# EvolEcolGroup/tidypopgen

Measured on AMD Instinct MI355X. Metric: SNP-genotypes/s (N x M) for IBS+KING+GRM+Fst+PCA; max |delta| vs CPU ref (cpu_baseline.parity), higher is better.
Workload: dtype fp4-e2m1 operands (exact integers, f32 accumulate) for the cross-products, the PCA Gram and the grouped counts, int8 (int32 accumulate) for the loadings, f64 for statistics

## Files before the change

include/tpg.h:

```cpp
#ifndef TPG_H
#define TPG_H

#include <stddef.h>
#include <stdint.h>

#ifdef __cplusplus
extern "C" {
#endif

#define TPG_OK 0
#define TPG_EINVAL 1
#define TPG_EHIP 2
#define TPG_EUNSUPPORTED 3
#define TPG_ENUMERIC 4

typedef struct tpg_ctx tpg_ctx;
typedef struct tpg_fbm tpg_fbm;
typedef struct tpg_view tpg_view;
typedef struct tpg_pairwise tpg_pairwise;
typedef struct tpg_comm tpg_comm;
typedef struct tpg_multi tpg_multi;

const char* tpg_last_error(void);
const char* tpg_version(void);
// ... 473 lines not shown
  int32_t* loci_counts;
  double* hwe_p;
  int32_t* grouped_counts;
  double* grouped_hwe_p;
  int32_t* indiv_counts;
} tpg_stream_qc_job;
int tpg_stream_qc(tpg_ctx* ctx, tpg_stream* s, const tpg_stream_qc_job* job, tpg_stream_report* report);

int tpg_pca_center_scale(tpg_ctx* ctx, const tpg_view* v, double* center, double* scale);
int tpg_pca_gram(tpg_ctx* ctx, const tpg_view* v, const double* center, const double* scale, double* K);
int tpg_pca_gram_add(tpg_ctx* ctx, const tpg_view* v, const double* center, const double* scale, double* K);
int tpg_pca_partial_svd(tpg_ctx* ctx, const tpg_view* v, int k, double* d, double* u, double* vload,
                        double* center, double* scale, double* square_frobenius);
int tpg_pca_random_svd(tpg_ctx* ctx, const tpg_view* v, int k, double tol, double* d, double* u, double* vload,
                       double* center, double* scale, double* square_frobenius);
int tpg_sym_eig_topk(tpg_ctx* ctx, const double* K, int64_t n, int k, double* lambda, double* U);
int tpg_pca_loadings(tpg_ctx* ctx, const tpg_view* v, const double* center, const double* scale,
                     const double* U, const double* d, int k, double* vload);
int tpg_fbm256_prod_and_rowSumsSq(tpg_ctx* ctx, const tpg_view* v, const double* center,
                                  const double* scale, const double* V, int K, double* XV, double* rss);
int tpg_square_frobenius(tpg_ctx* ctx, const tpg_view* v, const double* center, const double* scale,
                         double* out);
int tpg_fbm256_valid_prod(tpg_ctx* ctx, const tpg_view* v, const double* Tab, int K, double* out);

#define TPG_PCA_OP_TOL_FLOOR 1e-8
int tpg_pca_zt_prod(tpg_ctx* ctx, const tpg_view* v, const double* center, const double* scale, const double* Q, int b,
                    double* W);
int tpg_pca_z_prod(tpg_ctx* ctx, const tpg_view* v, const double* center, const double* scale, const double* W, int b,
                   double* Y);
int tpg_pca_random_svd_op(tpg_ctx* ctx, const tpg_view* v, int k, double tol, double* d, double* u, double* vload,
                          double* center, double* scale, double* square_frobenius, int* n_apply);
size_t tpg_pca_op_scratch_bytes(int64_t n, int64_t m, int k);
int tpg_pca_gram_route_fits(tpg_ctx* ctx, int64_t n, int k, int* fits);

#define TPG_PCADAPT_MAX_K 64
#define TPG_SELECT_TILE 1024
int64_t tpg_select_tile(void);
int tpg_col_median_mad(tpg_ctx* ctx, const double* X, int64_t rows, int ncols, int64_t ld, double* med, double* mad,
                       int64_t* n_finite);
int tpg_pcadapt_zscores(tpg_ctx* ctx, const tpg_view* v, const double* U, int K, double* z, int64_t* n_valid);
int tpg_robust_dist_ogk(tpg_ctx* ctx, const double* Z, int64_t m, int K, double* dist, double* center, double* cov,
                        double* basis, int64_t* n_valid);
int tpg_pchisq_log10_upper(tpg_ctx* ctx, const double* x, int64_t count, int df, double* out);
int tpg_qchisq_median(int df, double* out);
int tpg_pcadapt(tpg_ctx* ctx, const tpg_view* v, const double* U, int K, double* z, double* dist, double* stat, double* log10p,
                double* gc_lambda, int64_t* n_valid);

int tpg_view_select_loci(tpg_ctx* ctx, const tpg_view* v, const int64_t* idx0, int64_t count, tpg_view** out);
int tpg_qnorm_upper(double p, double* x);
int tpg_rollmean_weights(int radius, double* w);
int tpg_rollmean_segments(tpg_ctx* ctx, const double* x, int64_t m, const int64_t* seg_start, int64_t nseg, int radius,
                          double* out);
int tpg_medcouple(tpg_ctx* ctx, const double* x, int64_t count, double* mc);
#define TPG_TUKEY_REPORT_DOUBLES 7
int tpg_tukey_mc_up(tpg_ctx* ctx, const double* x, int64_t count, double alpha, double* report);
int tpg_pca_auto_svd(tpg_ctx* ctx, const tpg_view* v, const int32_t* chrom, const int64_t* hi, int k, double thr_r2, int roll_size,
                     double alpha_tukey, int64_t min_mac, int max_iter, void** out);
int64_t tpg_autosvd_count(const void* r);
int tpg_autosvd_iters(const void* r);
int tpg_autosvd_converged(const void* r);
int tpg_autosvd_fetch(const void* r, double* d, double* u, double* vload, double* center, double* scale, int64_t* idx0,
                      double* square_frobenius);
int tpg_autosvd_history(const void* r, int iter, int64_t* n_kept, int64_t* n_outliers, double* report);
int tpg_autosvd_outliers(const void* r, int iter, int64_t* pos0, int64_t* idx0);
int tpg_autosvd_intervals(const void* r, int iter, int64_t min_size, int64_t* first0, int64_t* last0, int64_t* count);
void tpg_autosvd_free(void* r);
// ... 61 lines not shown
```

tidypopgen_amd/_lib.py:

```python
from __future__ import annotations

import ctypes as C
import os

_HERE = os.path.dirname(os.path.abspath(__file__))
LIB_PATH = os.environ.get("TPG_LIB_PATH") or os.path.join(_HERE, "libtpg_hip.so")


class TpgError(RuntimeError):
    def __init__(self, code: int, msg: str):
        super().__init__(f"[tpg error {code}] {msg}")
        self.code = code


def build(force: bool = False) -> str:
    import subprocess

    csrc = os.path.join(_HERE, "csrc")
    cmd = ["make", "-C", csrc, "-j8", "-s"]
    if force:
        cmd.append("-B")
    subprocess.check_call(cmd)
    return LIB_PATH

# ... 246 lines not shown
    "tpg_multi_create": (ci, [ci, vp, vp]),
    "tpg_multi_destroy": (None, [vp]),
    "tpg_multi_ndev": (ci, [vp]),
    "tpg_multi_ctx": (vp, [vp, ci]),
    "tpg_multi_comm": (vp, [vp, ci]),
    "tpg_multi_pairwise": (ci, [vp, vp, i64, i64, vp, i64, vp, i64, ci, vp, vp, vp, vp]),
    "tpg_multi_grouped_alt_freq": (ci, [vp, vp, i64, i64, vp, i64, vp, i64, vp, vp, ci, vp, ci, vp]),
    "tpg_multi_pop_fst": (ci, [vp, vp, i64, i64, vp, i64, vp, i64, vp, vp, ci, vp, ci, vp, ci, ci, ci, vp, vp, vp]),
    "tpg_multi_pca_partial_svd": (ci, [vp, vp, i64, i64, vp, i64, vp, i64, vp, ci, vp, vp, vp, vp, vp, vp]),
    "tpg_stream_open_host": (ci, [vp, vp, i64, i64, sz, vp]),
    "tpg_stream_open_bk": (ci, [vp, cstr, i64, i64, sz, vp]),
    "tpg_stream_open_bed": (ci, [vp, cstr, i64, i64, sz, vp]),
    "tpg_stream_open_bed_host": (ci, [vp, vp, i64, i64, sz, vp]),
    "tpg_stream_open_synth": (ci, [vp, u64, i64, i64, ci, u32, ci, sz, vp]),
    "tpg_stream_close": (None, [vp]),
    "tpg_stream_run": (ci, [vp, vp, P(StreamJob), P(StreamReport)]),
    "tpg_multi_stream_run": (ci, [vp, vp, P(StreamJob), P(StreamReport)]),
    "tpg_stream_qc": (ci, [vp, vp, P(StreamQcJob), P(StreamReport)]),
    "tpg_pca_center_scale": (ci, [vp, vp, vp, vp]),
    "tpg_pca_gram": (ci, [vp, vp, vp, vp, vp]),
    "tpg_pca_gram_add": (ci, [vp, vp, vp, vp, vp]),
    "tpg_pca_partial_svd": (ci, [vp, vp, ci, vp, vp, vp, vp, vp, vp]),
    "tpg_pca_random_svd": (ci, [vp, vp, ci, f64, vp, vp, vp, vp, vp, vp]),
    "tpg_sym_eig_topk": (ci, [vp, vp, i64, ci, vp, vp]),
    "tpg_pca_loadings": (ci, [vp, vp, vp, vp, vp, vp, ci, vp]),
    "tpg_fbm256_prod_and_rowSumsSq": (ci, [vp, vp, vp, vp, vp, ci, vp, vp]),
    "tpg_square_frobenius": (ci, [vp, vp, vp, vp, vp]),
    "tpg_fbm256_valid_prod": (ci, [vp, vp, vp, ci, vp]),
    "tpg_pca_zt_prod": (ci, [vp, vp, vp, vp, vp, ci, vp]),
    "tpg_pca_z_prod": (ci, [vp, vp, vp, vp, vp, ci, vp]),
    "tpg_pca_random_svd_op": (ci, [vp, vp, ci, f64, vp, vp, vp, vp, vp, vp, vp]),
    "tpg_pca_op_scratch_bytes": (sz, [i64, i64, ci]),
    "tpg_pca_gram_route_fits": (ci, [vp, i64, ci, vp]),
    "tpg_select_tile": (i64, []),
    "tpg_col_median_mad": (ci, [vp, vp, i64, ci, i64, vp, vp, vp]),
    "tpg_pcadapt_zscores": (ci, [vp, vp, vp, ci, vp, vp]),
    "tpg_robust_dist_ogk": (ci, [vp, vp, i64, ci, vp, vp, vp, vp, vp]),
    "tpg_pchisq_log10_upper": (ci, [vp, vp, i64, ci, vp]),
    "tpg_qchisq_median": (ci, [ci, vp]),
    "tpg_pcadapt": (ci, [vp, vp, vp, ci, vp, vp, vp, vp, vp, vp]),
    "tpg_view_select_loci": (ci, [vp, vp, vp, i64, vp]),
    "tpg_qnorm_upper": (ci, [f64, vp]),
    "tpg_rollmean_weights": (ci, [ci, vp]),
    "tpg_rollmean_segments": (ci, [vp, vp, i64, vp, i64, ci, vp]),
    "tpg_medcouple": (ci, [vp, vp, i64, vp]),
    "tpg_tukey_mc_up": (ci, [vp, vp, i64, f64, vp]),
    "tpg_pca_auto_svd": (ci, [vp, vp, vp, vp, ci, f64, ci, f64, i64, ci, vp]),
    "tpg_autosvd_count": (i64, [vp]),
    "tpg_autosvd_iters": (ci, [vp]),
    "tpg_autosvd_converged": (ci, [vp]),
    "tpg_autosvd_fetch": (ci, [vp, vp, vp, vp, vp, vp, vp, vp]),
    "tpg_autosvd_history": (ci, [vp, ci, vp, vp, vp]),
    "tpg_autosvd_outliers": (ci, [vp, ci, vp, vp]),
    "tpg_autosvd_intervals": (ci, [vp, ci, i64, vp, vp, vp]),
    "tpg_autosvd_free": (None, [vp]),
    "tpg_kmeans_chunk_doubles": (i64, []),
    "tpg_kmeans_start": (ci, [u64, i64, ci, vp]),
    "tpg_kmeans_step": (ci, [vp, vp, i64, ci, ci, vp, vp, vp, vp, vp]),
    "tpg_kmeans_batch": (ci, [vp, vp, i64, ci, ci, vp, vp, ci, vp, vp, vp, vp, vp, vp, vp]),
    "tpg_cluster_wss": (ci, [vp, vp, i64, ci, ci, vp, vp, vp, vp]),
    "tpg_hclust_ward": (ci, [vp, vp, i64, ci, ci, vp, vp, vp]),
    "tpg_hclust_ward_trace": (ci, [vp, vp, i64, ci, ci, vp, vp, vp, vp]),
    "tpg_hclust_cut": (ci, [i64, vp, vp, ci, vp, vp]),
    "tpg_hclust_r_merge": (ci, [i64, vp, vp, vp]),
    "tpg_lda": (ci, [vp, i64, ci, vp, ci, ci, vp, vp, vp, vp, vp, vp, vp, vp, vp, vp, vp]),
    "tpg_dapc_var_contr": (ci, [vp, vp, i64, i64, ci, vp, ci, vp, vp]),
# ... 27 lines not shown
```

tidypopgen_amd/csrc/gramcls.hip:

```cpp
#include <math.h>
#include <string.h>

#include <algorithm>
#include <vector>

#include <hipcub/hipcub.hpp>

#include "common.h"
#include "devfrag.h"
#include "host/host_bits2.h"

constexpr int GA = 2, GB = 2, GP = GA * GB;
#define GCLS_SLAB (GP * 16 * 64)
#define GCLS_MAX_RUN 65536

__global__ void tpg_gcls_keys_kernel(const double* __restrict__ w, int64_t m, unsigned long long* __restrict__ key,
                                     uint32_t* __restrict__ idx) {
  for (int64_t j = blockIdx.x * (int64_t)blockDim.x + threadIdx.x; j < m; j += (int64_t)gridDim.x * blockDim.x) {
    const unsigned long long b = (unsigned long long)__double_as_longlong(w[j]);
    key[j] = (b + 16ull) & ~31ull;
    idx[j] = (uint32_t)j;
  }
}

__global__ void tpg_gcls_run_blocks_kernel(const uint32_t* __restrict__ counts, const int* __restrict__ nruns, int64_t m,
                                           uint32_t* __restrict__ cnt_out, uint32_t* __restrict__ nblk) {
  const int nr = nruns[0];
  for (int64_t r = blockIdx.x * (int64_t)blockDim.x + threadIdx.x; r < m; r += (int64_t)gridDim.x * blockDim.x) {
    const uint32_t c = r < nr ? counts[r] : 0u;
    cnt_out[r] = c;
    nblk[r] = (c + 63u) / 64u;
  }
}

__device__ __forceinline__ int tpg_gcls_find_run(const uint32_t* __restrict__ start, int nr, uint32_t x) {
  int lo = 0, hi = nr - 1;
  while (lo < hi) {
    const int mid = (lo + hi + 1) >> 1;
    if (start[mid] <= x) lo = mid; else hi = mid - 1;
  }
  return lo;
}

// ... 155 lines not shown
    __builtin_amdgcn_wave_barrier();
    __builtin_amdgcn_fence(__ATOMIC_ACQUIRE, "workgroup");
#pragma unroll
    for (int s = 0; s < 4; s++) {
      uint4 o = rd_dst[s * (2 * GSH_HS / 4)];
      if constexpr (CEN) {
        const uint32_t A[2] = {o.x, o.y}, B[2] = {o.z, o.w};
        uint32_t out[4];
#pragma unroll
        for (int t = 0; t < 2; t++) {
          const uint32_t nb = ~B[t], lo = nb & v55[t], hi = (nb >> 1) & lo, bc = lo | (hi << 1);
          out[2 * t] = (A[t] & 0x33333333u) | ((bc & 0x33333333u) << 2);
          out[2 * t + 1] = ((A[t] >> 2) & 0x33333333u) | (bc & 0xCCCCCCCCu);
        }
        o = make_uint4(out[0], out[1], out[2], out[3]);
      }
      T2g[((4 * q + s) * rs2 + bp) * 64 + lane] = o;
    }
    __builtin_amdgcn_fence(__ATOMIC_RELEASE, "workgroup");
    __builtin_amdgcn_wave_barrier();
    }
#pragma unroll
    for (int hb = 0; hb < 2; hb++) {
#pragma unroll
      for (int qi = 0; qi < QW; qi++) { w[qi][hb][0] = wn[qi][hb][0]; w[qi][hb][1] = wn[qi][hb][1]; }
      j0[hb] = j1[hb]; j1[hb] = j2[hb];
    }
  }
}

#define GCLS_SC_TWO ((int)0x80808080)

#define GCLS_D 2
__global__ __launch_bounds__(256, 2) void tpg_gcls_gram_kernel(const uint4* __restrict__ T2g, int64_t nblocks, int64_t rs2, int nrtv,
                                                               const unsigned long long* __restrict__ wblk,
                                                               const int2* __restrict__ order, int64_t nun, int S,
                                                               double* __restrict__ slabs) {
  constexpr int WPE = 2;
  const int lane = threadIdx.x & 63;
  const int wv = __builtin_amdgcn_readfirstlane(threadIdx.x >> 6);
  const int hgrid = gridDim.x / WPE, half = (int)blockIdx.x / hgrid, bx = (int)blockIdx.x % hgrid;
  const int xcd = bx & 7, cidx = bx >> 3, cpx = hgrid >> 3;
  const int SH = S / WPE;
  const int64_t npairs = (nblocks + 1) >> 1;
  for (int64_t round = 0;; round++) {
    const int64_t un = ((round * 8 + xcd) * cpx + cidx) * 4 + wv;
    if (un >= nun * SH) break;
    const int ks = half * SH + (int)(un / nun);
    const int64_t u = un % nun;
    const int2 ijv = order[u];
    const int2 ij = make_int2(__builtin_amdgcn_readfirstlane(ijv.x), __builtin_amdgcn_readfirstlane(ijv.y));
    const int64_t p0 = tpg_uniform64((npairs * ks) / S), p1 = tpg_uniform64((npairs * (ks + 1)) / S);
    const int64_t bend = 2 * p1 < nblocks ? 2 * p1 : nblocks;
    const uint4* pt[GA + GB];
#pragma unroll
    for (int t = 0; t < GA; t++) pt[t] = T2g + ((int64_t)min(GA * ij.x + t, nrtv - 1) * rs2) * 64;
#pragma unroll
    for (int t = 0; t < GB; t++) pt[GA + t] = T2g + ((int64_t)min(GB * ij.y + t, nrtv - 1) * rs2) * 64;

    double o[GP][16];
#pragma unroll
    for (int p = 0; p < GP; p++)
#pragma unroll
      for (int i = 0; i < 16; i++) o[p][i] = 0.0;
    v16f acc[GP];
#pragma unroll
    for (int p = 0; p < GP; p++)
#pragma unroll
      for (int i = 0; i < 16; i++) acc[p][i] = 0.f;

    if (p0 < p1) {
      const int64_t pl = p1 - 1, bl = bend - 1;
      v4u R[GCLS_D][GA + GB];
      auto LD = [&](const uint4* p) {
        uint32_t off = (uint32_t)lane * 16u;
        asm("" : "+v"(off));
        return *(const v4u*)((const char*)p + off);
      };
      tpg_static_for<GCLS_D - 1>([&](auto dd) {
        constexpr int d = decltype(dd)::value;
        const int64_t pc = p0 + d < p1 ? p0 + d : pl;
#pragma unroll
        for (int t = 0; t < GA + GB; t++) R[d][t] = LD(pt[t] + pc * 64);
      });
      bool first = true;
// ... 12 lines not shown
              const int64_t b = 2 * pr + hb;
              if (b < bend) {
                const unsigned long long wf = wf_next;
                wf_next = wblk[b < bl ? b + 1 : bl];
                v4u X[GA + GB];
#pragma unroll
                for (int t = 0; t < GA + GB; t++) {
                  const uint32_t w0 = R[C][t][2 * hb], w1 = R[C][t][2 * hb + 1];
                  X[t] = v4u{w0 & 0x33333333u, (w0 >> 2) & 0x33333333u, w1 & 0x33333333u, (w1 >> 2) & 0x33333333u};
                }
                if (first) {
                  const v16f z = {0, 0, 0, 0, 0, 0, 0, 0, 0, 0, 0, 0, 0, 0, 0, 0};
#pragma unroll
                  for (int p = 0; p < GP; p++) acc[p] = tpg_mfma_f4(X[p / GB], X[GA + p % GB], z, GCLS_SC_TWO, GCLS_SC_TWO);
                } else {
#pragma unroll
                  for (int p = 0; p < GP; p++) acc[p] = tpg_mfma_f4(X[p / GB], X[GA + p % GB], acc[p], GCLS_SC_TWO, GCLS_SC_TWO);
                }
                first = false;
                if ((wf & 1ull) || b == bl) {
                  const double w = __longlong_as_double((long long)(wf & ~1ull));
#pragma unroll
                  for (int p = 0; p < GP; p++)
#pragma unroll
                    for (int i = 0; i < 16; i++) o[p][i] = __builtin_fma((double)acc[p][i], w, o[p][i]);
                  first = true;
                }
              }
            }
          }
        });
      }
    }
    double* slab = slabs + ((int64_t)ks * nun + u) * GCLS_SLAB + lane;
#pragma unroll
    for (int p = 0; p < GP; p++)
#pragma unroll
      for (int i = 0; i < 16; i++) slab[(p * 16 + i) * 64] = o[p][i];
  }
}

typedef float v2f __attribute__((ext_vector_type(2)));
#define GCLS2_T_CLASS 0.045
#define GCLS2_T_BLOCK 0.067
#define GCLS2_LDS_BYTES (4 * 2 * 16 * 64 * 8)
#ifndef GCLS2_D
#define GCLS2_D 2
#endif
#define GCLS_SC_HALF ((int)0x7E7E7E7E)
template <bool CEN>
__global__ __launch_bounds__(256, 2) void tpg_gcls_gram2_kernel(const uint4* __restrict__ T2g, int64_t nblocks, int64_t rs2, int nrtv,
                                                                const ulonglong2* __restrict__ wblk,
                                                                const int2* __restrict__ order, int64_t nun, int S,
                                                                double* __restrict__ slabs) {
  extern __shared__ double olds_raw[];
  constexpr int WPE = 2;
  const int lane = threadIdx.x & 63;
  const int wv = __builtin_amdgcn_readfirstlane(threadIdx.x >> 6);
  double* olds = olds_raw + (size_t)wv * (2 * 16 * 64) + lane;
  const int hgrid = gridDim.x / WPE, half = (int)blockIdx.x / hgrid, bx = (int)blockIdx.x % hgrid;
  const int xcd = bx & 7, cidx = bx >> 3, cpx = hgrid >> 3;
  const int SH = S / WPE;
  const int64_t npairs = (nblocks + 1) >> 1;
  for (int64_t round = 0;; round++) {
    const int64_t un = ((round * 8 + xcd) * cpx + cidx) * 4 + wv;
    if (un >= nun * SH) break;
    const int ks = half * SH + (int)(un / nun);
    const int64_t u = un % nun;
    const int2 ijv = order[u];
    const int2 ij = make_int2(__builtin_amdgcn_readfirstlane(ijv.x), __builtin_amdgcn_readfirstlane(ijv.y));
    const int p0 = __builtin_amdgcn_readfirstlane((int)((npairs * ks) / S)), p1 = __builtin_amdgcn_readfirstlane((int)((npairs * (ks + 1)) / S));
    const int bend = 2 * p1;
    const char* pt[GA + GB];
#pragma unroll
    for (int t = 0; t < GA; t++) pt[t] = (const char*)(T2g + ((int64_t)min(GA * ij.x + t, nrtv - 1) * rs2 + p0) * 64);
#pragma unroll
    for (int t = 0; t < GB; t++) pt[GA + t] = (const char*)(T2g + ((int64_t)min(GB * ij.y + t, nrtv - 1) * rs2 + p0) * 64);

    double o[2][16];
    v2f dev[GP][8];
    v16f acc[GP];
#pragma unroll
    for (int p = 0; p < GP; p++) {
#pragma unroll
      for (int i = 0; i < 16; i++) acc[p][i] = 0.f;
#pragma unroll
      for (int i = 0; i < 8; i++) dev[p][i] = v2f{0.f, 0.f};
    }
#pragma unroll
    for (int p = 0; p < 2; p++)
#pragma unroll
      for (int i = 0; i < 16; i++) { o[p][i] = 0.0; olds[(p * 16 + i) * 64] = 0.0; }

    if (p0 < p1) {
      const int pl = p1 - 1, bl = bend - 1;
      v4u R[GCLS2_D][GA + GB];
      auto LDP = [&](v4u* slot, int pc) {
        uint32_t off = (uint32_t)lane * 16u + (uint32_t)(pc - p0) * 1024u;
        asm("" : "+v"(off));
#pragma unroll
        for (int t = 0; t < GA + GB; t++) slot[t] = *(const v4u*)(pt[t] + off);
      };
      tpg_static_for<GCLS2_D - 1>([&](auto dd) {
        constexpr int d = decltype(dd)::value;
// ... 84 lines not shown
                    for (int e = 0; e < 4; e++) dev[pr_][(e0 >> 1) + e] = dev[pl_][(e0 >> 1) + e] = v2f{0.f, 0.f};
                    __builtin_amdgcn_sched_barrier(0);
                  });
                } else {
                  pdelta = __uint_as_float((uint32_t)wf.y);
                  st = 2;
                }
                }
              }
            }
          }
        });
      }
      {
        const double w = __longlong_as_double((long long)(wlast & ~3ull));
        tpg_static_for<4>([&](auto hh) {
          constexpr int h = decltype(hh)::value, pr_ = h >> 1, pl_ = 2 + (h >> 1), e0 = (h & 1) * 8;
          double t[8];
#pragma unroll
          for (int e = 0; e < 8; e++) t[e] = olds[((pl_ - 2) * 16 + e0 + e) * 64];
#pragma unroll
          for (int e = 0; e < 8; e++) {
            const int i = e0 + e;
            o[pr_][i] = __builtin_fma((double)acc[pr_][i], w, o[pr_][i]) + (double)dev[pr_][i >> 1][i & 1];
          }
#pragma unroll
          for (int e = 0; e < 8; e++) {
            const int i = e0 + e;
            olds[((pl_ - 2) * 16 + i) * 64] = __builtin_fma((double)acc[pl_][i], w, t[e]) + (double)dev[pl_][i >> 1][i & 1];
          }
        });
      }
    }
    double* slab = slabs + ((int64_t)ks * nun + u) * GCLS_SLAB + lane;
#pragma unroll
    for (int p = 0; p < GP; p++)
#pragma unroll
      for (int i = 0; i < 16; i++) slab[(p * 16 + i) * 64] = p < 2 ? o[p][i] : olds[((p - 2) * 16 + i) * 64];
  }
}

__global__ __launch_bounds__(256) void tpg_gcls_assemble_kernel(const double* __restrict__ slabs, const int2* __restrict__ order,
                                                                int64_t nun, int S, int n, double* __restrict__ K) {
  __shared__ double tile[GP][32][33];
  const int lane = threadIdx.x & 63, wv = threadIdx.x >> 6;
  static_assert(GP == 4, "one wave per tile of the unit");
  for (int64_t u = blockIdx.x; u < nun; u += gridDim.x) {
    const int2 ij = order[u];
    const int p = wv;
    const int ti = GA * ij.x + p / GB, tk = GB * ij.y + p % GB;
    if (tk < ti) continue;
    double v[16];
#pragma unroll
    for (int reg = 0; reg < 16; reg++) v[reg] = 0.0;
    for (int s = 0; s < S; s++) {
      const double* sl = slabs + ((int64_t)s * nun + u) * GCLS_SLAB + (p * 16) * 64 + lane;
#pragma unroll
      for (int reg = 0; reg < 16; reg++) v[reg] += sl[reg * 64];
    }
#pragma unroll
    for (int reg = 0; reg < 16; reg++) tile[p][tpg_cd_row(reg, lane)][lane & 31] = v[reg];
    __builtin_amdgcn_fence(__ATOMIC_RELEASE, "workgroup");
    __builtin_amdgcn_wave_barrier();
    __builtin_amdgcn_fence(__ATOMIC_ACQUIRE, "workgroup");
    const int a = lane & 31, h = lane >> 5;
#pragma unroll 4
    for (int it = 0; it < 16; it++) {
      const int c = 2 * it + h;
      const int i1 = 32 * ti + a, k1 = 32 * tk + c;
      if (i1 < n && k1 < n) K[i1 + (int64_t)k1 * n] = tile[p][a][c];
      const int i2 = 32 * ti + c, k2 = 32 * tk + a;
      if (i2 < n && k2 < n) K[k2 + (int64_t)i2 * n] = tile[p][c][a];
    }
    __builtin_amdgcn_wave_barrier();
  }
}

static bool gcls_fold64(int64_t nruns, int64_t nblocks) {
  if (tpg_env_set("TPG_GRAM_FOLD64")) return tpg_env_int("TPG_GRAM_FOLD64", 0) != 0;
  return (double)nruns < 0.15 * (double)nblocks;
}

static double gcls_cost_classes(int64_t nunits, int64_t nruns, int64_t nblocks, int nwaves, int* bestS) {
  double best = -1;
  const bool f64 = gcls_fold64(nruns, nblocks);
  const double t_class = f64 ? 0.136 : GCLS2_T_CLASS, t_block = f64 ? 0.079 : GCLS2_T_BLOCK;
  for (int S = 2; S <= 32; S += 2) {
    if (nblocks / S < 4 && S > 2) break;
    const int64_t rounds = ceil_div(nunits * S, (int64_t)nwaves);
    const double per = ((double)nruns / S + 1.0) * GP * t_class + (double)ceil_div(nblocks, (int64_t)S) * GP * t_block + 6.0;
    const double cost = (double)rounds * per + (double)S * (double)nunits * 8.5e-3;
    if (best < 0 || cost < best * 0.995) { best = cost; *bestS = S; }
  }
  return best;
}

static int gram_classes_core(tpg_ctx* ctx, int64_t n, int64_t Q, int64_t m, const GclsSrc& src, const double* d_w, double* d_what,
                             double* d_K, bool force, bool* done, bool centred_ok) {
  *done = false;
  if (m >= (1ll << 31) - 64 || (tpg_env_set("TPG_GRAM_DIGITS") && !force)) return TPG_OK;
  DevArena B;
  unsigned long long *d_key = nullptr, *d_key2 = nullptr, *d_ukeys = nullptr;
  uint32_t *d_idx = nullptr, *d_idx2 = nullptr, *d_counts = nullptr, *d_cnt = nullptr, *d_nblk = nullptr, *d_estart = nullptr,
           *d_bstart = nullptr;
  int* d_nruns = nullptr;
  long long* d_totals = nullptr;
  void* d_tmp = nullptr;
  TPG_TRY(B.get(&d_key, (size_t)m)); TPG_TRY(B.get(&d_key2, (size_t)m)); TPG_TRY(B.get(&d_ukeys, (size_t)m));
  TPG_TRY(B.get(&d_idx, (size_t)m)); TPG_TRY(B.get(&d_idx2, (size_t)m)); TPG_TRY(B.get(&d_counts, (size_t)m));
  TPG_TRY(B.get(&d_cnt, (size_t)m)); TPG_TRY(B.get(&d_nblk, (size_t)m)); TPG_TRY(B.get(&d_estart, (size_t)m));
  TPG_TRY(B.get(&d_bstart, (size_t)m)); TPG_TRY(B.get(&d_nruns, 1)); TPG_TRY(B.get(&d_totals, 2));
  size_t t_sort = 0, t_rle = 0, t_scan = 0;
  TPG_HIP(hipcub::DeviceRadixSort::SortPairs(nullptr, t_sort, d_key, d_key2, d_idx, d_idx2, (int)m, 0, 64, ctx->stream));
  TPG_HIP(hipcub::DeviceRunLengthEncode::Encode(nullptr, t_rle, d_key2, d_ukeys, d_counts, d_nruns, (int)m, ctx->stream));
  TPG_HIP(hipcub::DeviceScan::ExclusiveSum(nullptr, t_scan, d_cnt, d_estart, (int)m, ctx->stream));
  const size_t t_bytes = std::max(t_sort, std::max(t_rle, t_scan));
  TPG_TRY(B.get((uint8_t**)&d_tmp, t_bytes));
  long long totals[2] = {0, 0};
  {
    ProfScope ps(ctx, "gcls_classes");
    hipLaunchKernelGGL(tpg_gcls_keys_kernel, dim3(1024), dim3(256), 0, ctx->stream, d_w, m, d_key, d_idx);
    size_t t = t_bytes;
    TPG_HIP(hipcub::DeviceRadixSort::SortPairs(d_tmp, t, d_key, d_key2, d_idx, d_idx2, (int)m, 0, 64, ctx->stream));
    t = t_bytes;
    TPG_HIP(hipcub::DeviceRunLengthEncode::Encode(d_tmp, t, d_key2, d_ukeys, d_counts, d_nruns, (int)m, ctx->stream));
    hipLaunchKernelGGL(tpg_gcls_run_blocks_kernel, dim3(1024), dim3(256), 0, ctx->stream, (const uint32_t*)d_counts,
                       (const int*)d_nruns, m, d_cnt, d_nblk);
    t = t_bytes;
    TPG_HIP(hipcub::DeviceScan::ExclusiveSum(d_tmp, t, d_cnt, d_estart, (int)m, ctx->stream));
    t = t_bytes;
    TPG_HIP(hipcub::DeviceScan::ExclusiveSum(d_tmp, t, d_nblk, d_bstart, (int)m, ctx->stream));
    hipLaunchKernelGGL(tpg_gcls_totals_kernel, dim3(1), dim3(1), 0, ctx->stream, (const int*)d_nruns,
                       (const uint32_t*)d_bstart, (const uint32_t*)d_nblk, d_totals);
  }
  TPG_HIP(tpg_fetch_small(ctx, totals, d_totals, sizeof(totals)));
  const int64_t nruns = totals[0], nblocks = totals[1];
  TPG_REQUIRE(nruns > 0 && nblocks > 0, TPG_EHIP, "class table is empty");

  const int nrtv = (int)ceil_div(n, 32);
  const int nI = (int)ceil_div(nrtv, GA), nJ = (int)ceil_div(nrtv, GB);
  std::vector<int2> order;
  const int PJ = 8;
  for (int pj = 0; pj * PJ < nJ; pj++) {
    const int j1 = std::min(nJ, pj * PJ + PJ);
    for (int I = 0; I < nI; I++)
      for (int J = pj * PJ; J < j1; J++)
        if (GB * J + GB - 1 >= GA * I) order.push_back(make_int2(I, J));
  }
  const int64_t nun = (int64_t)order.size();
  int ncu8 = ctx->num_cu / 8 * 8;
  if (ncu8 < 8) ncu8 = 8;
  const bool f64 = gcls_fold64(nruns, nblocks);
  static const bool no_cen = tpg_env_int("TPG_GRAM_CENTER", 1) == 0;
  const bool cen = centred_ok && !no_cen && !f64;
  const int nblk_grid = 2 * ncu8;
  const int nwaves = 4 * nblk_grid;
  int S = 2;
  const double cost_cls = gcls_cost_classes(nun, nruns, nblocks, nwaves, &S) + 350.0 + 1.25e-3 * (double)m * ((double)n / 5000.0);
  const int64_t nun_dig = (int64_t)nrtv * ceil_div((int64_t)nrtv, 4) / 2 + nrtv;
  const int t_dig = std::max(4, ((int)ceil(log2(2.0 * (double)n + 1.0)) + ctx->pca_digit_fbits + 7) / 7);
  const double cost_dig = (double)ceil_div(nun_dig, (int64_t)(4 * ncu8)) * ((double)ceil_div(m, 128) * 0.25 * t_dig) + 65.0;
  while ((nblocks / 2 + S) / S + 2 >= (1 << 21)) S += 2;
  if (tpg_env_set("TPG_DEBUG"))
    fprintf(stderr, "[tpg] gram classes: %lld classes, %lld blocks for %lld loci, S = %d, model %.0f us (digits %.0f us)\n",
            (long long)nruns, (long long)nblocks, (long long)m, S, cost_cls, cost_dig);
  if (cost_cls > cost_dig && !force && !tpg_env_set("TPG_GRAM_CLASSES")) return TPG_OK;

  int32_t* d_src = nullptr;
  double* d_slabs = nullptr;
  unsigned long long* d_wblk = nullptr;
  ulonglong2* d_wblk2 = nullptr;
  uint4* d_T2g = nullptr;
  int2* d_order = nullptr;
  TPG_TRY(B.get(&d_src, (size_t)nblocks * 64));
  if (f64) TPG_TRY(B.get(&d_wblk, (size_t)nblocks));
  else TPG_TRY(B.get(&d_wblk2, (size_t)nblocks + 4));
  const int64_t rs2 = (nblocks + 1) / 2;
  TPG_TRY(B.get(&d_T2g, (size_t)(4 * Q) * (size_t)rs2 * 64));
  TPG_TRY(B.get(&d_order, (size_t)nun));
  TPG_TRY(B.get(&d_slabs, (size_t)S * (size_t)nun * GCLS_SLAB));
  TPG_HIP(tpg_h2d_async(ctx, d_order, order.data(), sizeof(int2) * (size_t)nun));
  TPG_HIP(hipMemsetAsync(d_src, 0xFF, sizeof(int32_t) * (size_t)nblocks * 64, ctx->stream));
  {
    ProfScope ps(ctx, "gcls_layout");
    hipLaunchKernelGGL(tpg_gcls_place_kernel, dim3(1024), dim3(256), 0, ctx->stream, (const uint32_t*)d_idx2,
                       (const unsigned long long*)d_ukeys, (const uint32_t*)d_estart, (const uint32_t*)d_bstart, (int)nruns, m,
                       d_src, d_what);
    if (f64)
      hipLaunchKernelGGL(tpg_gcls_block_table_kernel, dim3(256), dim3(256), 0, ctx->stream, (const unsigned long long*)d_ukeys,
                         (const uint32_t*)d_bstart, (const uint32_t*)d_nblk, (int)nruns, nblocks, d_wblk);
    else
      hipLaunchKernelGGL(tpg_gcls_block_table2_kernel, dim3(256), dim3(256), 0, ctx->stream, (const unsigned long long*)d_ukeys,
                         (const uint32_t*)d_bstart, (const uint32_t*)d_nblk, (int)nruns, nblocks, GCLS_GMAX, GCLS_GQ, d_wblk2);
  }
  {
    const int64_t tasks = Q * rs2;
    if (tasks >= ((int64_t)1 << 31)) return TPG_OK;
    const unsigned grid = (unsigned)std::min<int64_t>(ceil_div(tasks, 4), (int64_t)ctx->num_cu * 16);
    const int qw = tpg_env_int("TPG_GATHER_QW", Q >= 4 ? 4 : Q >= 2 ? 2 : 1);
#define GATHER_GO(C, W) TPG_LAUNCH(ctx, "gcls_gather", (tpg_gcls_gather_kernel<C, W>), dim3(grid), dim3(256), 0, src, Q, (const int32_t*)d_src, nblocks, rs2, d_T2g)
    if (cen) { if (qw == 4) GATHER_GO(true, 4); else if (qw == 2) GATHER_GO(true, 2); else GATHER_GO(true, 1); }
    else { if (qw == 4) GATHER_GO(false, 4); else if (qw == 2) GATHER_GO(false, 2); else GATHER_GO(false, 1); }
#undef GATHER_GO
  }
  if (f64)
    TPG_LAUNCH(ctx, "pca_gram_classes", tpg_gcls_gram_kernel, dim3((unsigned)nblk_grid), dim3(256), 0, (const uint4*)d_T2g, nblocks,
               rs2, nrtv, (const unsigned long long*)d_wblk, (const int2*)d_order, nun, S, d_slabs);
  else if (cen) {
    (void)hipFuncSetAttribute((const void*)tpg_gcls_gram2_kernel<true>, hipFuncAttributeMaxDynamicSharedMemorySize, GCLS2_LDS_BYTES);
    TPG_LAUNCH(ctx, "pca_gram_classes", tpg_gcls_gram2_kernel<true>, dim3((unsigned)nblk_grid), dim3(256), GCLS2_LDS_BYTES,
               (const uint4*)d_T2g, nblocks, rs2, nrtv, (const ulonglong2*)d_wblk2, (const int2*)d_order, nun, S, d_slabs);
  } else {
    (void)hipFuncSetAttribute((const void*)tpg_gcls_gram2_kernel<false>, hipFuncAttributeMaxDynamicSharedMemorySize, GCLS2_LDS_BYTES);
    TPG_LAUNCH(ctx, "pca_gram_classes", tpg_gcls_gram2_kernel<false>, dim3((unsigned)nblk_grid), dim3(256), GCLS2_LDS_BYTES,
               (const uint4*)d_T2g, nblocks, rs2, nrtv, (const ulonglong2*)d_wblk2, (const int2*)d_order, nun, S, d_slabs);
  }
  TPG_LAUNCH(ctx, "gcls_assemble", tpg_gcls_assemble_kernel, dim3((unsigned)std::min<int64_t>(nun, 4096)), dim3(256), 0,
             (const double*)d_slabs, (const int2*)d_order, nun, S, (int)n, d_K);
  TPG_CHECK_LAUNCH();
  *done = true;
  return TPG_OK;
}

__global__ __launch_bounds__(256) void tpg_gcls_l2lm_kernel(const uint4* __restrict__ L, int64_t Q, int64_t n_lt,
                                                            uint4* __restrict__ LM) {
  __shared__ uint4 sh[32][8];
  for (int64_t task = blockIdx.x; task < tpg_lm_tasks(n_lt, Q); task += gridDim.x) {
    TpgLmSide l, lm;
    tpg_lm_task(task, Q, (int)threadIdx.x, l, lm);
    if (l.on) sh[l.row][l.col] = L[l.piece];
    __syncthreads();
    if (lm.on) LM[lm.piece] = sh[lm.row][lm.col];
    __syncthreads();
  }
}

int tpg_gram_classes(tpg_ctx* ctx, const tpg_view* v, const double* d_w, double* d_what, double* d_K, bool* done,
                     bool centred_ok) {
  *done = false;
  if (tpg_env_set("TPG_GRAM_DIGITS")) return TPG_OK;
  const int64_t n_lt = 4 * v->KG;
  DevBuf d_LM;
  if (!v->LM) {
    TPG_TRY(tpg_view_need_L(ctx, v));
    TPG_TRY(d_LM.alloc_n<uint4>((size_t)n_lt * 32 * (size_t)v->Q * 2));
    TPG_LAUNCH(ctx, "gcls_l2lm", tpg_gcls_l2lm_kernel, dim3((unsigned)std::min<int64_t>(n_lt * ((v->Q + 3) / 4), (int64_t)ctx->num_cu * 32)),
               dim3(256), 0, (const uint4*)v->L, v->Q, n_lt, d_LM.as<uint4>());
  }
  const GclsSrc src{v->LM ? v->LM : d_LM.as<uint4>(), 0, 2 * v->Q, 0, 0, 2, 1};
  const int rc = gram_classes_core(ctx, v->n, v->Q, v->m, src, d_w, d_what, d_K, false, done, centred_ok);
  d_LM.free();
  return rc;
}
// ... 188 lines not shown
```

Baseline: 144.5 billion.

## Replace uniform split-K grid with a host-planned item table for class Gram

The class-based PCA Gram kernels used to split every output unit into the same number S of block ranges, which leaves a partial last round of waves. A host planner now picks the total number of work items so that they fill whole rounds of waves. It allows units to have different split counts and packs items into a table that each wave reads by slot. The assemble kernel sums a per-unit list of slabs, so each unit can have a different slab count. The cost is an extra host-to-device upload of the plan tables and host planning work on every call, in exchange for less tail idle time.

Result: no change. 145.0 billion (median of 5 runs) (+0.4%).

```diff
diff --git a/include/tpg.h b/include/tpg.h
--- a/include/tpg.h
+++ b/include/tpg.h
@@ -529,6 +529,8 @@
                           double* center, double* scale, double* square_frobenius, int* n_apply);
 size_t tpg_pca_op_scratch_bytes(int64_t n, int64_t m, int k);
 int tpg_pca_gram_route_fits(tpg_ctx* ctx, int64_t n, int k, int* fits);
+int tpg_gram_plan(tpg_ctx* ctx, int64_t n, int64_t nruns, int64_t nblocks, int workgroups, int fold64, int64_t* sizes,
+                  int32_t* units, int32_t* items, int32_t* slab_first, int32_t* slab_list);
 
 #define TPG_PCADAPT_MAX_K 64
 #define TPG_SELECT_TILE 1024
diff --git a/tidypopgen_amd/_lib.py b/tidypopgen_amd/_lib.py
--- a/tidypopgen_amd/_lib.py
+++ b/tidypopgen_amd/_lib.py
@@ -302,6 +302,7 @@
     "tpg_pca_random_svd_op": (ci, [vp, vp, ci, f64, vp, vp, vp, vp, vp, vp, vp]),
     "tpg_pca_op_scratch_bytes": (sz, [i64, i64, ci]),
     "tpg_pca_gram_route_fits": (ci, [vp, i64, ci, vp]),
+    "tpg_gram_plan": (ci, [vp, i64, i64, i64, ci, ci, vp, vp, vp, vp, vp]),
     "tpg_select_tile": (i64, []),
     "tpg_col_median_mad": (ci, [vp, vp, i64, ci, i64, vp, vp, vp]),
     "tpg_pcadapt_zscores": (ci, [vp, vp, vp, ci, vp, vp]),
diff --git a/tidypopgen_amd/csrc/gramcls.hip b/tidypopgen_amd/csrc/gramcls.hip
--- a/tidypopgen_amd/csrc/gramcls.hip
+++ b/tidypopgen_amd/csrc/gramcls.hip
@@ -9,6 +9,7 @@
 #include "common.h"
 #include "devfrag.h"
 #include "host/host_bits2.h"
+#include "host/host_gramplan.h"
 
 constexpr int GA = 2, GB = 2, GP = GA * GB;
 #define GCLS_SLAB (GP * 16 * 64)
@@ -230,25 +231,32 @@
 #define GCLS_SC_TWO ((int)0x80808080)
 
 #define GCLS_D 2
+struct GclsItem {
+  int unit, p0, p1, slab;
+};
+__device__ __forceinline__ GclsItem gcls_item(const int4* __restrict__ items, int64_t i) {
+  uint32_t off = 0;
+  asm("" : "+v"(off));
+  const int4 v = *(const int4*)((const char*)(items + i) + off);
+  return GclsItem{__builtin_amdgcn_readfirstlane(v.x), __builtin_amdgcn_readfirstlane(v.y), __builtin_amdgcn_readfirstlane(v.z),
+                  __builtin_amdgcn_readfirstlane(v.w)};
+}
 __global__ __launch_bounds__(256, 2) void tpg_gcls_gram_kernel(const uint4* __restrict__ T2g, int64_t nblocks, int64_t rs2, int nrtv,
                                                                const unsigned long long* __restrict__ wblk,
-                                                               const int2* __restrict__ order, int64_t nun, int S,
-                                                               double* __restrict__ slabs) {
+                                                               const int2* __restrict__ order, const int4* __restrict__ items,
+                                                               int nrounds, double* __restrict__ slabs) {
   constexpr int WPE = 2;
   const int lane = threadIdx.x & 63;
   const int wv = __builtin_amdgcn_readfirstlane(threadIdx.x >> 6);
   const int hgrid = gridDim.x / WPE, half = (int)blockIdx.x / hgrid, bx = (int)blockIdx.x % hgrid;
   const int xcd = bx & 7, cidx = bx >> 3, cpx = hgrid >> 3;
-  const int SH = S / WPE;
-  const int64_t npairs = (nblocks + 1) >> 1;
-  for (int64_t round = 0;; round++) {
-    const int64_t un = ((round * 8 + xcd) * cpx + cidx) * 4 + wv;
-    if (un >= nun * SH) break;
-    const int ks = half * SH + (int)(un / nun);
-    const int64_t u = un % nun;
-    const int2 ijv = order[u];
+  const int slot = ((half * 8 + xcd) * cpx + cidx) * 4 + wv, nwv = (int)gridDim.x * 4;
+  for (int round = 0; round < nrounds; round++) {
+    const GclsItem it = gcls_item(items, (int64_t)round * nwv + slot);
+    if (it.unit < 0) break;
+    const int2 ijv = order[it.unit];
     const int2 ij = make_int2(__builtin_amdgcn_readfirstlane(ijv.x), __builtin_amdgcn_readfirstlane(ijv.y));
-    const int64_t p0 = tpg_uniform64((npairs * ks) / S), p1 = tpg_uniform64((npairs * (ks + 1)) / S);
+    const int64_t p0 = it.p0, p1 = it.p1;
     const int64_t bend = 2 * p1 < nblocks ? 2 * p1 : nblocks;
     const uint4* pt[GA + GB];
 #pragma unroll
@@ -327,7 +335,7 @@
         });
       }
     }
-    double* slab = slabs + ((int64_t)ks * nun + u) * GCLS_SLAB + lane;
+    double* slab = slabs + (int64_t)it.slab * GCLS_SLAB + lane;
 #pragma unroll
     for (int p = 0; p < GP; p++)
 #pragma unroll
@@ -346,8 +354,8 @@
 template <bool CEN>
 __global__ __launch_bounds__(256, 2) void tpg_gcls_gram2_kernel(const uint4* __restrict__ T2g, int64_t nblocks, int64_t rs2, int nrtv,
                                                                 const ulonglong2* __restrict__ wblk,
-                                                                const int2* __restrict__ order, int64_t nun, int S,
-                                                                double* __restrict__ slabs) {
+                                                                const int2* __restrict__ order, const int4* __restrict__ items,
+                                                                int nrounds, double* __restrict__ slabs) {
   extern __shared__ double olds_raw[];
   constexpr int WPE = 2;
   const int lane = threadIdx.x & 63;
@@ -355,16 +363,13 @@
   double* olds = olds_raw + (size_t)wv * (2 * 16 * 64) + lane;
   const int hgrid = gridDim.x / WPE, half = (int)blockIdx.x / hgrid, bx = (int)blockIdx.x % hgrid;
   const int xcd = bx & 7, cidx = bx >> 3, cpx = hgrid >> 3;
-  const int SH = S / WPE;
-  const int64_t npairs = (nblocks + 1) >> 1;
-  for (int64_t round = 0;; round++) {
-    const int64_t un = ((round * 8 + xcd) * cpx + cidx) * 4 + wv;
-    if (un >= nun * SH) break;
-    const int ks = half * SH + (int)(un / nun);
-    const int64_t u = un % nun;
-    const int2 ijv = order[u];
+  const int slot = ((half * 8 + xcd) * cpx + cidx) * 4 + wv, nwv = (int)gridDim.x * 4;
+  for (int round = 0; round < nrounds; round++) {
+    const GclsItem it = gcls_item(items, (int64_t)round * nwv + slot);
+    if (it.unit < 0) break;
+    const int2 ijv = order[it.unit];
     const int2 ij = make_int2(__builtin_amdgcn_readfirstlane(ijv.x), __builtin_amdgcn_readfirstlane(ijv.y));
-    const int p0 = __builtin_amdgcn_readfirstlane((int)((npairs * ks) / S)), p1 = __builtin_amdgcn_readfirstlane((int)((npairs * (ks + 1)) / S));
+    const int p0 = it.p0, p1 = it.p1;
     const int bend = 2 * p1;
     const char* pt[GA + GB];
 #pragma unroll
@@ -515,7 +520,7 @@
         });
       }
     }
-    double* slab = slabs + ((int64_t)ks * nun + u) * GCLS_SLAB + lane;
+    double* slab = slabs + (int64_t)it.slab * GCLS_SLAB + lane;
 #pragma unroll
     for (int p = 0; p < GP; p++)
 #pragma unroll
@@ -524,7 +529,8 @@
 }
 
 __global__ __launch_bounds__(256) void tpg_gcls_assemble_kernel(const double* __restrict__ slabs, const int2* __restrict__ order,
-                                                                int64_t nun, int S, int n, double* __restrict__ K) {
+                                                                const int* __restrict__ slab_first, const int* __restrict__ slab_list,
+                                                                int64_t nun, int n, double* __restrict__ K) {
   __shared__ double tile[GP][32][33];
   const int lane = threadIdx.x & 63, wv = threadIdx.x >> 6;
   static_assert(GP == 4, "one wave per tile of the unit");
@@ -536,8 +542,9 @@
     double v[16];
 #pragma unroll
     for (int reg = 0; reg < 16; reg++) v[reg] = 0.0;
-    for (int s = 0; s < S; s++) {
-      const double* sl = slabs + ((int64_t)s * nun + u) * GCLS_SLAB + (p * 16) * 64 + lane;
+    const int s1 = slab_first[u + 1];
+    for (int s = slab_first[u]; s < s1; s++) {
+      const double* sl = slabs + (int64_t)slab_list[s] * GCLS_SLAB + (p * 16) * 64 + lane;
 #pragma unroll
       for (int reg = 0; reg < 16; reg++) v[reg] += sl[reg * 64];
     }
@@ -564,18 +571,42 @@
   return (double)nruns < 0.15 * (double)nblocks;
 }
 
-static double gcls_cost_classes(int64_t nunits, int64_t nruns, int64_t nblocks, int nwaves, int* bestS) {
-  double best = -1;
-  const bool f64 = gcls_fold64(nruns, nblocks);
-  const double t_class = f64 ? 0.136 : GCLS2_T_CLASS, t_block = f64 ? 0.079 : GCLS2_T_BLOCK;
-  for (int S = 2; S <= 32; S += 2) {
-    if (nblocks / S < 4 && S > 2) break;
-    const int64_t rounds = ceil_div(nunits * S, (int64_t)nwaves);
-    const double per = ((double)nruns / S + 1.0) * GP * t_class + (double)ceil_div(nblocks, (int64_t)S) * GP * t_block + 6.0;
-    const double cost = (double)rounds * per + (double)S * (double)nunits * 8.5e-3;
-    if (best < 0 || cost < best * 0.995) { best = cost; *bestS = S; }
-  }
-  return best;
+static GramPlanCost gcls_plan_cost(bool f64) {
+  return GramPlanCost{f64 ? 0.136 : GCLS2_T_CLASS, f64 ? 0.079 : GCLS2_T_BLOCK, 6.0, 8.5e-3};
+}
+static double gcls_cost_classes(int64_t nunits, int64_t nruns, int64_t nblocks, int nwaves, int64_t* nitems) {
+  const int rounds = tpg_env_int("TPG_GRAM_ROUNDS", 0);
+  double cost = 0.0;
+  *nitems = gramplan_items(nunits, nruns, nblocks, nwaves, gcls_plan_cost(gcls_fold64(nruns, nblocks)),
+                           rounds > 0 ? (int64_t)rounds * nwaves : 0, &cost);
+  return cost;
+}
+
+static int gcls_gram_grid(int num_cu) {
+  int ncu8 = num_cu / 8 * 8;
+  if (ncu8 < 8) ncu8 = 8;
+  int grid = 2 * ncu8;
+  const int want = tpg_env_int("TPG_GRAM_GRID", 0);
+  if (want > 0) grid = std::min(grid, std::max(16, want / 16 * 16));
+  return grid;
+}
+
+static void gcls_unit_order(int64_t n, std::vector<int2>* order) {
+  const int nrtv = (int)ceil_div(n, 32);
+  const int nI = (int)ceil_div(nrtv, GA), nJ = (int)ceil_div(nrtv, GB);
+  const int PJ = 8;
+  for (int pj = 0; pj * PJ < nJ; pj++) {
+    const int j1 = std::min(nJ, pj * PJ + PJ);
+    for (int I = 0; I < nI; I++)
+      for (int J = pj * PJ; J < j1; J++)
+        if (GB * J + GB - 1 >= GA * I) order->push_back(make_int2(I, J));
+  }
+}
+
+static int gcls_h2d_pieces(tpg_ctx* ctx, void* d_dst, const void* src, size_t bytes) {
+  for (size_t o = 0; o < bytes; o += tpg_ctx::H2D_SLOT_BYTES)
+    TPG_HIP(tpg_h2d_async(ctx, (uint8_t*)d_dst + o, (const uint8_t*)src + o, std::min(bytes - o, tpg_ctx::H2D_SLOT_BYTES)));
+  return TPG_OK;
 }
 
 static int gram_classes_core(tpg_ctx* ctx, int64_t n, int64_t Q, int64_t m, const GclsSrc& src, const double* d_w, double* d_what,
@@ -621,32 +652,24 @@
   TPG_REQUIRE(nruns > 0 && nblocks > 0, TPG_EHIP, "class table is empty");
 
   const int nrtv = (int)ceil_div(n, 32);
-  const int nI = (int)ceil_div(nrtv, GA), nJ = (int)ceil_div(nrtv, GB);
   std::vector<int2> order;
-  const int PJ = 8;
-  for (int pj = 0; pj * PJ < nJ; pj++) {
-    const int j1 = std::min(nJ, pj * PJ + PJ);
-    for (int I = 0; I < nI; I++)
-      for (int J = pj * PJ; J < j1; J++)
-        if (GB * J + GB - 1 >= GA * I) order.push_back(make_int2(I, J));
-  }
+  gcls_unit_order(n, &order);
   const int64_t nun = (int64_t)order.size();
   int ncu8 = ctx->num_cu / 8 * 8;
   if (ncu8 < 8) ncu8 = 8;
   const bool f64 = gcls_fold64(nruns, nblocks);
   static const bool no_cen = tpg_env_int("TPG_GRAM_CENTER", 1) == 0;
   const bool cen = centred_ok && !no_cen && !f64;
-  const int nblk_grid = 2 * ncu8;
+  const int nblk_grid = gcls_gram_grid(ctx->num_cu);
   const int nwaves = 4 * nblk_grid;
-  int S = 2;
-  const double cost_cls = gcls_cost_classes(nun, nruns, nblocks, nwaves, &S) + 350.0 + 1.25e-3 * (double)m * ((double)n / 5000.0);
+  int64_t nitems = 0;
+  const double cost_cls = gcls_cost_classes(nun, nruns, nblocks, nwaves, &nitems) + 350.0 + 1.25e-3 * (double)m * ((double)n / 5000.0);
   const int64_t nun_dig = (int64_t)nrtv * ceil_div((int64_t)nrtv, 4) / 2 + nrtv;
   const int t_dig = std::max(4, ((int)ceil(log2(2.0 * (double)n + 1.0)) + ctx->pca_digit_fbits + 7) / 7);
   const double cost_dig = (double)ceil_div(nun_dig, (int64_t)(4 * ncu8)) * ((double)ceil_div(m, 128) * 0.25 * t_dig) + 65.0;
-  while ((nblocks / 2 + S) / S + 2 >= (1 << 21)) S += 2;
   if (tpg_env_set("TPG_DEBUG"))
-    fprintf(stderr, "[tpg] gram classes: %lld classes, %lld blocks for %lld loci, S = %d, model %.0f us (digits %.0f us)\n",
-            (long long)nruns, (long long)nblocks, (long long)m, S, cost_cls, cost_dig);
+    fprintf(stderr, "[tpg] gram classes: %lld classes, %lld blocks for %lld loci, %d rounds of %d waves, %lld items = slabs, model %.0f us (digits %.0f us)\n",
+            (long long)nruns, (long long)nblocks, (long long)m, gramplan_rounds(nitems, nwaves), nwaves, (long long)nitems, cost_cls, cost_dig);
   if (cost_cls > cost_dig && !force && !tpg_env_set("TPG_GRAM_CLASSES")) return TPG_OK;
 
   int32_t* d_src = nullptr;
@@ -655,13 +678,18 @@
   ulonglong2* d_wblk2 = nullptr;
   uint4* d_T2g = nullptr;
   int2* d_order = nullptr;
+  int4* d_items = nullptr;
+  int *d_sfirst = nullptr, *d_slist = nullptr;
   TPG_TRY(B.get(&d_src, (size_t)nblocks * 64));
   if (f64) TPG_TRY(B.get(&d_wblk, (size_t)nblocks));
   else TPG_TRY(B.get(&d_wblk2, (size_t)nblocks + 4));
   const int64_t rs2 = (nblocks + 1) / 2;
   TPG_TRY(B.get(&d_T2g, (size_t)(4 * Q) * (size_t)rs2 * 64));
   TPG_TRY(B.get(&d_order, (size_t)nun));
-  TPG_TRY(B.get(&d_slabs, (size_t)S * (size_t)nun * GCLS_SLAB));
+  TPG_TRY(B.get(&d_slabs, (size_t)nitems * GCLS_SLAB));
+  TPG_TRY(B.get(&d_items, (size_t)gramplan_rounds(nitems, nwaves) * (size_t)nwaves));
+  TPG_TRY(B.get(&d_sfirst, (size_t)nun + 1));
+  TPG_TRY(B.get(&d_slist, (size_t)nitems));
   TPG_HIP(tpg_h2d_async(ctx, d_order, order.data(), sizeof(int2) * (size_t)nun));
   TPG_HIP(hipMemsetAsync(d_src, 0xFF, sizeof(int32_t) * (size_t)nblocks * 64, ctx->stream));
   {
@@ -686,22 +714,52 @@
     else { if (qw == 4) GATHER_GO(false, 4); else if (qw == 2) GATHER_GO(false, 2); else GATHER_GO(false, 1); }
 #undef GATHER_GO
   }
+  GramPlan plan;
+  gramplan_deal(nun, nblocks, nwaves, nitems, &plan);
+  static_assert(sizeof(GramPlanItem) == sizeof(int4), "the kernels read an item as one int4");
+  TPG_TRY(gcls_h2d_pieces(ctx, d_items, plan.table.data(), sizeof(GramPlanItem) * plan.table.size()));
+  TPG_TRY(gcls_h2d_pieces(ctx, d_sfirst, plan.slab_first.data(), sizeof(int32_t) * plan.slab_first.size()));
+  TPG_TRY(gcls_h2d_pieces(ctx, d_slist, plan.slab_list.data(), sizeof(int32_t) * plan.slab_list.size()));
   if (f64)
     TPG_LAUNCH(ctx, "pca_gram_classes", tpg_gcls_gram_kernel, dim3((unsigned)nblk_grid), dim3(256), 0, (const uint4*)d_T2g, nblocks,
-               rs2, nrtv, (const unsigned long long*)d_wblk, (const int2*)d_order, nun, S, d_slabs);
+               rs2, nrtv, (const unsigned long long*)d_wblk, (const int2*)d_order, (const int4*)d_items, plan.rounds, d_slabs);
   else if (cen) {
     (void)hipFuncSetAttribute((const void*)tpg_gcls_gram2_kernel<true>, hipFuncAttributeMaxDynamicSharedMemorySize, GCLS2_LDS_BYTES);
     TPG_LAUNCH(ctx, "pca_gram_classes", tpg_gcls_gram2_kernel<true>, dim3((unsigned)nblk_grid), dim3(256), GCLS2_LDS_BYTES,
-               (const uint4*)d_T2g, nblocks, rs2, nrtv, (const ulonglong2*)d_wblk2, (const int2*)d_order, nun, S, d_slabs);
+               (const uint4*)d_T2g, nblocks, rs2, nrtv, (const ulonglong2*)d_wblk2, (const int2*)d_order, (const int4*)d_items, plan.rounds, d_slabs);
   } else {
     (void)hipFuncSetAttribute((const void*)tpg_gcls_gram2_kernel<false>, hipFuncAttributeMaxDynamicSharedMemorySize, GCLS2_LDS_BYTES);
     TPG_LAUNCH(ctx, "pca_gram_classes", tpg_gcls_gram2_kernel<false>, dim3((unsigned)nblk_grid), dim3(256), GCLS2_LDS_BYTES,
-               (const uint4*)d_T2g, nblocks, rs2, nrtv, (const ulonglong2*)d_wblk2, (const int2*)d_order, nun, S, d_slabs);
+               (const uint4*)d_T2g, nblocks, rs2, nrtv, (const ulonglong2*)d_wblk2, (const int2*)d_order, (const int4*)d_items, plan.rounds, d_slabs);
   }
   TPG_LAUNCH(ctx, "gcls_assemble", tpg_gcls_assemble_kernel, dim3((unsigned)std::min<int64_t>(nun, 4096)), dim3(256), 0,
-             (const double*)d_slabs, (const int2*)d_order, nun, S, (int)n, d_K);
+             (const double*)d_slabs, (const int2*)d_order, (const int*)d_sfirst, (const int*)d_slist, nun, (int)n, d_K);
   TPG_CHECK_LAUNCH();
   *done = true;
+  return TPG_OK;
+}
+
+extern "C" int tpg_gram_plan(tpg_ctx* ctx, int64_t n, int64_t nruns, int64_t nblocks, int workgroups, int fold64, int64_t* sizes,
+                             int32_t* units, int32_t* items, int32_t* slab_first, int32_t* slab_list) {
+  TPG_REQUIRE((ctx || workgroups > 0) && sizes && n > 0 && nruns > 0 && nblocks > 0 && nblocks < (1ll << 31) && workgroups >= 0 && workgroups % 16 == 0,
+              TPG_EINVAL, "bad argument");
+  std::vector<int2> order;
+  gcls_unit_order(n, &order);
+  const int64_t nun = (int64_t)order.size();
+  const int nwaves = 4 * (workgroups ? workgroups : gcls_gram_grid(ctx->num_cu));
+  const bool f64 = fold64 < 0 ? gcls_fold64(nruns, nblocks) : fold64 != 0;
+  double cost = 0.0;
+  const int rounds_env = tpg_env_int("TPG_GRAM_ROUNDS", 0);
+  const int64_t nitems = gramplan_items(nun, nruns, nblocks, nwaves, gcls_plan_cost(f64), rounds_env > 0 ? (int64_t)rounds_env * nwaves : 0, &cost);
+  sizes[0] = nun; sizes[1] = nwaves; sizes[2] = gramplan_rounds(nitems, nwaves); sizes[3] = nitems;
+  if (!items) return TPG_OK;
+  TPG_REQUIRE(units && slab_first && slab_list, TPG_EINVAL, "null argument");
+  GramPlan plan;
+  gramplan_deal(nun, nblocks, nwaves, nitems, &plan);
+  memcpy(units, order.data(), sizeof(int2) * (size_t)nun);
+  memcpy(items, plan.table.data(), sizeof(GramPlanItem) * plan.table.size());
+  memcpy(slab_first, plan.slab_first.data(), sizeof(int32_t) * plan.slab_first.size());
+  memcpy(slab_list, plan.slab_list.data(), sizeof(int32_t) * plan.slab_list.size());
   return TPG_OK;
 }
 
diff --git a/tidypopgen_amd/csrc/host/host_gramplan.h b/tidypopgen_amd/csrc/host/host_gramplan.h
--- /dev/null
+++ b/tidypopgen_amd/csrc/host/host_gramplan.h
@@ -0,0 +1,159 @@
+#pragma once
+#include <stdint.h>
+
+#include <algorithm>
+#include <vector>
+
+struct GramPlanItem {
+  int32_t unit, p0, p1, slab;
+};
+
+struct GramPlanCost {
+  double t_class, t_block, t_item, t_slab;
+};
+
+struct GramPlan {
+  int64_t nitems = 0;
+  int rounds = 0;
+  std::vector<GramPlanItem> table;
+  std::vector<int32_t> slab_first;
+  std::vector<int32_t> slab_list;
+};
+
+static const int GRAMPLAN_TILES = 4;
+
+struct GramPlanRun {
+  int64_t u0, u1;
+  int a0, a1;
+};
+
+static inline int gramplan_runs(int64_t nun, int64_t N, GramPlanRun runs[3]) {
+  const int64_t N0 = (N + 1) / 2, N1 = N / 2;
+  const int q0 = (int)(N0 / nun), q1 = (int)(N1 / nun);
+  const int64_t x0 = N0 % nun, y1 = nun - N1 % nun;
+  const int64_t cut[4] = {0, std::min(x0, y1), std::max(x0, y1), nun};
+  int nr = 0;
+  for (int i = 0; i < 3; i++) {
+    if (cut[i] == cut[i + 1]) continue;
+    runs[nr++] = GramPlanRun{cut[i], cut[i + 1], q0 + (cut[i] < x0 ? 1 : 0), q1 + (cut[i] >= y1 ? 1 : 0)};
+  }
+  return nr;
+}
+
+static inline double gramplan_item_cost(int64_t nruns, int64_t nblocks, int c, const GramPlanCost& C) {
+  return ((double)nruns / c + 1.0) * GRAMPLAN_TILES * C.t_class + ((double)nblocks / c) * GRAMPLAN_TILES * C.t_block + C.t_item;
+}
+
+static inline double gramplan_cost(int64_t nun, int64_t nruns, int64_t nblocks, int nwaves, int64_t N, const GramPlanCost& C) {
+  GramPlanRun runs[3];
+  const int nr = gramplan_runs(nun, N, runs);
+  const int64_t W = nwaves / 2;
+  double worst = 0.0;
+  for (int h = 0; h < 2; h++) {
+    int64_t cnt[3];
+    int cc[3], idx[3] = {0, 1, 2};
+    for (int i = 0; i < nr; i++) {
+      cc[i] = runs[i].a0 + runs[i].a1;
+      cnt[i] = (runs[i].u1 - runs[i].u0) * (h ? runs[i].a1 : runs[i].a0);
+    }
+    for (int i = 0; i < nr; i++)
+      for (int j = i + 1; j < nr; j++)
+        if (cc[idx[j]] < cc[idx[i]]) std::swap(idx[i], idx[j]);
+    double wave = 0.0;
+    int64_t pos = 0, seen = 0;
+    for (int i = 0; i < nr; i++) {
+      seen += cnt[idx[i]];
+      for (; pos < seen; pos += W) wave += gramplan_item_cost(nruns, nblocks, cc[idx[i]], C);
+    }
+    worst = std::max(worst, wave);
+  }
+  return worst + (double)N * C.t_slab;
+}
+
+static inline void gramplan_limits(int64_t nblocks, int* cmin, int* cmax) {
+  const int64_t npairs = (nblocks + 1) / 2;
+  const int64_t lo = (npairs + ((1 << 21) - 5)) / ((1 << 21) - 4);
+  int64_t hi = std::min<int64_t>(32, std::max<int64_t>(nblocks / 4, std::min<int64_t>(2, npairs)));
+  if (hi < lo) hi = lo;
+  *cmin = (int)lo;
+  *cmax = (int)hi;
+}
+
+static inline int64_t gramplan_choose(int64_t nun, int64_t nruns, int64_t nblocks, int nwaves, const GramPlanCost& C, double* cost) {
+  int cmin, cmax;
+  gramplan_limits(nblocks, &cmin, &cmax);
+  const int64_t lo = nun * cmin, hi = nun * cmax;
+  double best = -1.0;
+  int64_t bestN = lo;
+  auto take = [&](int64_t N) {
+    const double c = gramplan_cost(nun, nruns, nblocks, nwaves, N, C);
+    if (best < 0 || c < best * 0.995) { best = c; bestN = N; }
+  };
+  take(lo);
+  for (int64_t N = (lo / nwaves + 1) * (int64_t)nwaves; N < hi; N += nwaves) take(N);
+  if (hi > lo) take(hi);
+  if (cost) *cost = best;
+  return bestN;
+}
+
+static inline void gramplan_deal(int64_t nun, int64_t nblocks, int nwaves, int64_t N, GramPlan* P) {
+  const int64_t npairs = (nblocks + 1) / 2, W = nwaves / 2;
+  GramPlanRun runs[3];
+  const int nr = gramplan_runs(nun, N, runs);
+  P->nitems = N;
+  P->rounds = (int)(((N + 1) / 2 + W - 1) / W);
+  P->table.assign((size_t)P->rounds * (size_t)nwaves, GramPlanItem{-1, 0, 0, -1});
+  P->slab_first.resize((size_t)nun + 1);
+  P->slab_list.resize((size_t)N);
+  int64_t s = 0;
+  for (int i = 0; i < nr; i++)
+    for (int64_t u = runs[i].u0; u < runs[i].u1; u++) { P->slab_first[(size_t)u] = (int32_t)s; s += runs[i].a0 + runs[i].a1; }
+  P->slab_first[(size_t)nun] = (int32_t)s;
+  for (int64_t i = 0; i < N; i++) P->slab_list[(size_t)i] = (int32_t)i;
+  int cs[3];
+  int ncs = 0;
+  for (int i = 0; i < nr; i++) cs[ncs++] = runs[i].a0 + runs[i].a1;
+  std::sort(cs, cs + ncs);
+  ncs = (int)(std::unique(cs, cs + ncs) - cs);
+  for (int h = 0; h < 2; h++) {
+    int64_t pos = 0;
+    std::vector<int32_t> cu, ca;
+    for (int ci = 0; ci < ncs; ci++) {
+      const int c = cs[ci];
+      cu.clear();
+      ca.clear();
+      for (int i = 0; i < nr; i++)
+        if (runs[i].a0 + runs[i].a1 == c)
+          for (int64_t u = runs[i].u0; u < runs[i].u1; u++) { cu.push_back((int32_t)u); ca.push_back(h ? runs[i].a1 : runs[i].a0); }
+      for (size_t g0 = 0; g0 < cu.size(); g0 += (size_t)W) {
+        const size_t g1 = std::min(cu.size(), g0 + (size_t)W);
+        int amax = 0;
+        for (size_t j = g0; j < g1; j++) amax = std::max(amax, (int)ca[j]);
+        for (int kl = 0; kl < amax; kl++)
+          for (size_t j = g0; j < g1; j++) {
+            if (ca[j] <= kl) continue;
+            const int32_t u = cu[j];
+            const int k = (h ? c - ca[j] : 0) + kl;
+            P->table[(size_t)((pos / W) * nwaves + h * W + pos % W)] =
+                GramPlanItem{u, (int32_t)(npairs * k / c), (int32_t)(npairs * (k + 1) / c), P->slab_first[(size_t)u] + k};
+            pos++;
+          }
+      }
+    }
+  }
+}
+
+static inline int64_t gramplan_items(int64_t nun, int64_t nruns, int64_t nblocks, int nwaves, const GramPlanCost& C, int64_t want,
+                                     double* cost) {
+  if (want <= 0) return gramplan_choose(nun, nruns, nblocks, nwaves, C, cost);
+  int cmin, cmax;
+  gramplan_limits(nblocks, &cmin, &cmax);
+  const int64_t N = std::min(std::max(want, nun * cmin), nun * cmax);
+  if (cost) *cost = gramplan_cost(nun, nruns, nblocks, nwaves, N, C);
+  return N;
+}
+
+static inline int gramplan_rounds(int64_t N, int nwaves) {
+  const int64_t W = nwaves / 2;
+  return (int)(((N + 1) / 2 + W - 1) / W);
+}
```
